# wmeddie/CycloneML

Measured on AMD Instinct MI355X. Metric: rows/s per training iteration, higher is better.
Workload: dtype f64

## Files before the change

### cycloneml_amd/csrc/kmeans.hip

```cpp
#pragma clang fp contract(off)

#include <hip/hip_runtime.h>

#include <algorithm>
#include <cmath>
#include <cstdlib>
#include <mutex>
#include <utility>
#include <vector>

#include "common.hpp"
#include "kmeans_i8.hpp"
#include "kmeans_cos.hpp"
#include "kmeans_fp64.hpp"
#include "kmeans_sparse.hpp"
#include "kmeans_sums.hpp"
#include "silhouette.hpp"

namespace {

using cyc::kmsums::kChunkRows;
using cyc::kmsums::kMaxK;

bool env_is0(const char* name) {
// ... 908 lines not shown
  CYC_REQUIRE(p != nullptr && out != nullptr, "plan and out must not be null");
  CYC_REQUIRE(n >= 0, "n >= 0");
  CYC_REQUIRE(X != nullptr || n == 0, "X must not be null");
  auto* r = new cyc_kmeans_rows_s();
  r->X = X;
  r->n = n;
  r->d = p->d;
  r->usable = p->d <= cyc::km8::kMaxD && p->ktp8 > 0;
  r->cosine = is_cos(p);
  if (r->usable && n > 0) {
    int rc;
    hipStream_t st = cyc::as_stream(stream);
    if ((rc = r->img.reserve((size_t)n * cyc::km8::image_row_bytes(p->d))) ||
        (rc = r->meta.reserve(sizeof(int2) * (size_t)n))) {
      delete r;
      return rc;
    }
    if (r->cosine) {
      cyc::DeviceBuffer xn;
      if ((rc = r->unorm.reserve(sizeof(double) * (size_t)n)) ||
          (rc = xn.reserve(sizeof(double) * (size_t)n))) {
        delete r;
        return rc;
      }
      hipLaunchKernelGGL(k_row_norms, dim3((unsigned)((n + kNormRows - 1) / kNormRows)),
                         dim3(kNormRows), 0, st, X, n, p->d, (double*)xn.ptr);
      CYC_LAUNCH_CHECK("k_row_norms");
      rc = cyc::km8::rows_quantize(X, n, p->d, r->img.ptr, (int2*)r->meta.ptr, st,
                                   (const double*)xn.ptr, (double*)r->unorm.ptr);
      if (!rc && hipStreamSynchronize(st) != hipSuccess) rc = CYC_ERR_HIP;
    } else {
      if ((rc = r->unorm.reserve(sizeof(double) * (size_t)n))) {
        delete r;
        return rc;
      }
      rc = cyc::km8::rows_quantize(X, n, p->d, r->img.ptr, (int2*)r->meta.ptr, st, nullptr,
                                   (double*)r->unorm.ptr);
    }
    if (rc) {
      delete r;
      return rc;
    }
  }
  *out = r;
  return CYC_OK;
}

int cyc_kmeans_rows_destroy(cyc_kmeans_rows rows) {
  delete rows;
  return CYC_OK;
}

int64_t cyc_kmeans_rows_bytes(cyc_kmeans_rows rows) {
  return rows ? (int64_t)(rows->img.bytes + rows->meta.bytes) : 0;
}

int cyc_kmeans_rows_set_bounds(cyc_kmeans_rows rows, int32_t enable) {
  CYC_REQUIRE(rows != nullptr, "rows must not be null");
  rows->bEnabled = enable != 0;
  rows->bValid = false;
  return CYC_OK;
}

int cyc_kmeans_rows_set_incremental(cyc_kmeans_rows rows, int32_t enable) {
  CYC_REQUIRE(rows != nullptr, "rows must not be null");
  rows->inc.enabled = enable != 0;
  rows->inc.valid = false;
  return CYC_OK;
}

int cyc_kmeans_rows_incremental_info(cyc_kmeans_rows rows, int64_t* incremental_calls,
                                     int64_t* moved_rows) {
  CYC_REQUIRE(rows != nullptr && incremental_calls != nullptr && moved_rows != nullptr,
              "arguments must not be null");
  unsigned long long cum[2] = {0, 0};
  if (rows->inc.cum.ptr) {
    CYC_HIP(hipDeviceSynchronize());
    CYC_HIP(hipMemcpy(cum, rows->inc.cum.ptr, sizeof(cum), hipMemcpyDeviceToHost));
  }
  *incremental_calls = (int64_t)cum[1];
  *moved_rows = (int64_t)cum[0];
  return CYC_OK;
}

int cyc_kmeans_rows_bounds_rechecked(cyc_kmeans_rows rows, int64_t* rechecked_rows) {
  CYC_REQUIRE(rows != nullptr && rechecked_rows != nullptr, "arguments must not be null");
  unsigned long long cum = 0;
  if (rows->bRcCum.ptr) {
    CYC_HIP(hipDeviceSynchronize());
    CYC_HIP(hipMemcpy(&cum, rows->bRcCum.ptr, sizeof(cum), hipMemcpyDeviceToHost));
  }
  *rechecked_rows = (int64_t)cum;
  return CYC_OK;
}

int cyc_kmeans_rows_bounds_info(cyc_kmeans_rows rows, int64_t* calls, int64_t* screened_rows) {
  CYC_REQUIRE(rows != nullptr && calls != nullptr && screened_rows != nullptr,
              "arguments must not be null");
  unsigned long long cum = 0;
  if (rows->bCum.ptr) {
    CYC_HIP(hipDeviceSynchronize());
    CYC_HIP(hipMemcpy(&cum, rows->bCum.ptr, sizeof(cum), hipMemcpyDeviceToHost));
  }
  *calls = rows->bCalls;
  *screened_rows = rows->bFullRows + (int64_t)cum;
  return CYC_OK;
}
// ... 420 lines not shown
```

### cycloneml_amd/csrc/kmeans_sums.hip

```cpp
#pragma clang fp contract(off)

#include <hip/hip_runtime.h>

#include <algorithm>
#include <type_traits>

#include "common.hpp"
#include "kmeans_cos.hpp"
#include "kmeans_sums.hpp"

namespace {

constexpr int kSortTile = 4096;
using cyc::kmsums::kChunkRows;

__global__ void k_hist(const int32_t* __restrict__ assign, int64_t n, int k,
                       int32_t* __restrict__ hist, const int* __restrict__ gate) {
  if (gate && !*gate) return;
  extern __shared__ int32_t cnt[];
  for (int c = threadIdx.x; c < k; c += blockDim.x) cnt[c] = 0;
  __syncthreads();
  const int64_t r0 = (int64_t)blockIdx.x * kSortTile;
  const int64_t r1 = min<int64_t>(n, r0 + kSortTile);
  for (int64_t r = r0 + threadIdx.x; r < r1; r += blockDim.x) atomicAdd(&cnt[assign[r]], 1);
  __syncthreads();
  for (int c = threadIdx.x; c < k; c += blockDim.x) hist[(int64_t)blockIdx.x * k + c] = cnt[c];
}

constexpr int kScanSegs = 64;

__global__ void k_scan_seg(const int32_t* __restrict__ hist, int tiles, int k, int segT,
                           int32_t* __restrict__ segsum, const int* __restrict__ gate) {
  if (gate && !*gate) return;
  const int c = blockIdx.x * 64 + threadIdx.x, s = blockIdx.y;
  if (c >= k) return;
  const int t0 = s * segT, t1 = min(tiles, t0 + segT);
  int sum = 0;
#pragma unroll 8
  for (int t = t0; t < t1; ++t) sum += hist[(int64_t)t * k + c];
  segsum[(int64_t)s * k + c] = sum;
}

__global__ void k_scan_segoff(int32_t* __restrict__ segsum, int segs, int k,
                              int64_t* __restrict__ total, const int* __restrict__ gate) {
  if (gate && !*gate) return;
  const int c = blockIdx.x * blockDim.x + threadIdx.x;
  if (c >= k) return;
  int64_t run = 0;
  for (int s = 0; s < segs; ++s) {
    const int32_t h = segsum[(int64_t)s * k + c];
    segsum[(int64_t)s * k + c] = (int32_t)run;
    run += h;
  }
  total[c] = run;
}

__global__ void k_scan_apply(int32_t* __restrict__ hist, int tiles, int k, int segT,
                             const int32_t* __restrict__ segoff, const int* __restrict__ gate) {
  if (gate && !*gate) return;
  const int c = blockIdx.x * 64 + threadIdx.x, s = blockIdx.y;
  if (c >= k) return;
  const int t0 = s * segT, t1 = min(tiles, t0 + segT);
  int32_t run = segoff[(int64_t)s * k + c];
  for (int t = t0; t < t1; ++t) {
    const int32_t h = hist[(int64_t)t * k + c];
    hist[(int64_t)t * k + c] = run;
    run += h;
  }
}

__global__ void k_scan_clusters(const int64_t* __restrict__ total, int k,
                                int64_t* __restrict__ cstart, int64_t* __restrict__ chunkStart,
                                const int* __restrict__ gate) {
  if (gate && !*gate) return;
  __shared__ int64_t s_rows[1024], s_chunks[1024];
  const int tid = threadIdx.x;
  const int per = (k + 1023) / 1024;
  int64_t rows = 0, chunks = 0;
  for (int q = 0; q < per; ++q) {
    int c = tid * per + q;
    if (c < k) {
      rows += total[c];
      chunks += (total[c] + kChunkRows - 1) / kChunkRows;
    }
  }
  s_rows[tid] = rows;
  s_chunks[tid] = chunks;
  __syncthreads();
  for (int off = 1; off < 1024; off <<= 1) {
    int64_t a = tid >= off ? s_rows[tid - off] : 0, b = tid >= off ? s_chunks[tid - off] : 0;
    __syncthreads();
    s_rows[tid] += a;
    s_chunks[tid] += b;
    __syncthreads();
  }
  int64_t rbase = tid ? s_rows[tid - 1] : 0, cbase = tid ? s_chunks[tid - 1] : 0;
  for (int q = 0; q < per; ++q) {
    int c = tid * per + q;
    if (c < k) {
      cstart[c] = rbase;
      chunkStart[c] = cbase;
      rbase += total[c];
      cbase += (total[c] + kChunkRows - 1) / kChunkRows;
    }
  }
  if (tid == 1023) {
    cstart[k] = s_rows[1023];
    chunkStart[k] = s_chunks[1023];
  }
}

__global__ void k_scatter(const int32_t* __restrict__ assign, int64_t n, int k,
                          const int32_t* __restrict__ tileOff, const int64_t* __restrict__ cstart,
                          int32_t* __restrict__ perm, int64_t tiles, const int* __restrict__ gate) {
  if (gate && !*gate) return;
  extern __shared__ int64_t pos[];
  const int64_t per = ((int64_t)gridDim.x + 7) / 8;
  const int64_t tile = (int64_t)(blockIdx.x & 7) * per + (blockIdx.x >> 3);
  if (tile >= tiles) return;
  const int lane = threadIdx.x;
  const int kb = 32 - __builtin_clz((unsigned)max(k - 1, 1));
  for (int c = lane; c < k; c += 64) pos[c] = cstart[c] + tileOff[tile * k + c];
  __syncthreads();
  const int64_t r0 = tile * kSortTile;
  const int64_t r1 = min<int64_t>(n, r0 + kSortTile);
  constexpr int PER = kSortTile / 64;
  int cv[PER];
#pragma unroll
  for (int i = 0; i < PER; ++i) {
    const int64_t r = r0 + i * 64 + lane;
    cv[i] = (r < r1) ? assign[r] : -1;
  }
#pragma unroll
  for (int i = 0; i < PER; ++i) {
    const int64_t r = r0 + i * 64 + lane;
    const int c = cv[i];
    unsigned long long m = __ballot(c >= 0);
    for (int b = 0; b < kb; ++b) {
      const bool bit = (c >> b) & 1;
      const unsigned long long bal = __ballot(bit);
      m &= bit ? bal : ~bal;
    }
    const int prior = __popcll(m & ((1ull << lane) - 1));
    const int last = 63 - __clzll(m);
    int64_t p = (c >= 0) ? pos[c] + prior : 0;
    __builtin_amdgcn_wave_barrier();
    if (c >= 0) {
      perm[p] = (int32_t)r;
      if (last == lane) pos[c] = p + 1;
    }
    __builtin_amdgcn_wave_barrier();
  }
}

template <int NJ>
__global__ __launch_bounds__(256) void k_chunk_sums(
    const double* __restrict__ X, int d, const double* __restrict__ w,
    const double* __restrict__ C, const int32_t* __restrict__ perm,
    const int64_t* __restrict__ cstart, const int64_t* __restrict__ chunkStart, int k,
    double* __restrict__ part, double* __restrict__ pw, double* __restrict__ pc,
    double* __restrict__ costOut) {
// ... 147 lines not shown
      for (int i = 0; i < cnt; ++i) sw = dadd(sw, w[rowsS[i]]);
    } else {
      sw = (double)cnt;
    }
    pw[ch] = sw;
    pc[ch] = red[0];
    if (pa) pa[ch] = reda[0];
  }
}

__global__ void k_chunk_sums_nocost(const double* __restrict__ X, int d,
                                    const double* __restrict__ w,
                                    const double* __restrict__ cost,
                                    const int32_t* __restrict__ perm,
                                    const int64_t* __restrict__ cstart,
                                    const int64_t* __restrict__ chunkStart, int k,
                                    double* __restrict__ part, double* __restrict__ pw,
                                    double* __restrict__ pc) {
  const int64_t ch = blockIdx.x;
  if (ch >= chunkStart[k]) return;
  int lo = 0, hi = k;
  while (hi - lo > 1) {
    int mid = (lo + hi) >> 1;
    if (chunkStart[mid] <= ch) lo = mid; else hi = mid;
  }
  const int c = lo;
  const int64_t first = cstart[c] + (ch - chunkStart[c]) * kChunkRows;
  const int64_t last = min<int64_t>(cstart[c + 1], first + kChunkRows);
  for (int j = threadIdx.x; j < d; j += blockDim.x) {
    double s = 0.0;
    if (w) {
      for (int64_t p = first; p < last; ++p) {
        const int64_t r = perm[p];
        s = dadd(s, dmul(w[r], X[r * d + j]));
      }
    } else {
      for (int64_t p = first; p < last; ++p) s = dadd(s, X[(int64_t)perm[p] * d + j]);
    }
    part[ch * d + j] = s;
  }
  if (threadIdx.x == 0) {
    double sw = 0.0, sc = 0.0;
    for (int64_t p = first; p < last; ++p) {
      const int64_t r = perm[p];
      const double wt = w ? w[r] : 1.0;
      sw = dadd(sw, wt);
      sc = dadd(sc, dmul(cost[r], wt));
    }
    pw[ch] = sw;
    pc[ch] = sc;
  }
}

__global__ void k_reduce_clusters(const double* __restrict__ part, const double* __restrict__ pw,
                                  const double* __restrict__ pc,
                                  const int64_t* __restrict__ chunkStart, int d,
                                  double* __restrict__ sums, double* __restrict__ wsum,
                                  double* __restrict__ ccost, const double* __restrict__ pa,
                                  double* __restrict__ fS, double* __restrict__ fW,
                                  double* __restrict__ fA, const int* __restrict__ gate) {
  if (gate && !*gate) return;
  const int c = blockIdx.x;
  const int64_t a = chunkStart[c], b = chunkStart[c + 1];
  if (a == b) {
    if (threadIdx.x == 0) ccost[c] = 0.0;
    if (fS) {
      for (int j = threadIdx.x; j < d; j += blockDim.x) fS[(int64_t)c * d + j] = 0.0;
      if (threadIdx.x == 0) fW[c] = fA[c] = 0.0;
    }
    return;
  }
  for (int j = threadIdx.x; j < d; j += blockDim.x) {
    double s = 0.0;
    int64_t ch = a;
    for (; ch + 16 <= b; ch += 16) {
      double v[16];
#pragma unroll
      for (int u = 0; u < 16; ++u) v[u] = part[(ch + u) * d + j];
#pragma unroll
      for (int u = 0; u < 16; ++u) s = dadd(s, v[u]);
    }
    for (; ch < b; ++ch) s = dadd(s, part[ch * d + j]);
    sums[(int64_t)c * d + j] = dadd(sums[(int64_t)c * d + j], s);
    if (fS) fS[(int64_t)c * d + j] = s;
  }
  const int tw = 64 % blockDim.x, tc = 128 % blockDim.x, ta = 192 % blockDim.x;
  if (fS && threadIdx.x == ta && ta != tw && ta != tc) {
    double s = 0.0;
    for (int64_t ch = a; ch < b; ++ch) s = dadd(s, pa[ch]);
    fA[c] = s;
  }
  if (threadIdx.x == tw || threadIdx.x == tc) {
    const double* src = threadIdx.x == tw ? pw : pc;
    double s = 0.0;
    int64_t ch = a;
    for (; ch + 8 <= b; ch += 8) {
      double v[8];
#pragma unroll
      for (int u = 0; u < 8; ++u) v[u] = src[ch + u];
#pragma unroll
      for (int u = 0; u < 8; ++u) s = dadd(s, v[u]);
    }
    for (; ch < b; ++ch) s = dadd(s, src[ch]);
    if (threadIdx.x == tw) {
      wsum[c] = dadd(wsum[c], s);
      if (fS) fW[c] = s;
    } else {
      ccost[c] = s;
    }
  }
}

__global__ void k_cost_total(const double* __restrict__ ccost, int k, double* __restrict__ out,
                             const int* __restrict__ gate) {
  if (gate && !*gate) return;
  __shared__ double s[256];
  double a = 0.0;
  for (int c = threadIdx.x; c < k; c += 256) a = dadd(a, ccost[c]);
  s[threadIdx.x] = a;
  __syncthreads();
  for (int off = 128; off > 0; off >>= 1) {
    if (threadIdx.x < off) s[threadIdx.x] = dadd(s[threadIdx.x], s[threadIdx.x + off]);
    __syncthreads();
  }
  if (threadIdx.x == 0) out[0] = dadd(out[0], s[0]);
}

constexpr int kIncRows = 2048;
constexpr int kIncMovedFrac = 16;

__global__ __launch_bounds__(256) void k_inc_moved(const int32_t* __restrict__ assign,
                                                   int32_t* __restrict__ prev, int64_t n,
                                                   int32_t* __restrict__ tmpRow,
                                                   int32_t* __restrict__ tmpOld,
                                                   unsigned int* __restrict__ bcount) {
  constexpr int IT = kIncRows / 256;
  __shared__ unsigned wc[IT * 4];
  const int tid = threadIdx.x, lane = tid & 63, wave = tid >> 6;
  const int64_t base = (int64_t)blockIdx.x * kIncRows;
  unsigned long long masks[IT];
  int32_t olds[IT];
#pragma unroll
  for (int it = 0; it < IT; ++it) {
    const int64_t r = base + it * 256 + tid;
    bool moved = false;
    olds[it] = -1;
    if (r < n) {
      const int32_t a = assign[r], b = prev[r];
      moved = a != b;
      olds[it] = b;
      if (moved) prev[r] = a;
    }
    masks[it] = __builtin_amdgcn_ballot_w64(moved);
    if (lane == 0) wc[it * 4 + wave] = (unsigned)__builtin_popcountll(masks[it]);
  }
  __syncthreads();
  const unsigned long long below = (1ull << lane) - 1ull;
#pragma unroll
  for (int it = 0; it < IT; ++it) {
    unsigned before = 0;
    for (int j = 0; j < it * 4 + wave; ++j) before += wc[j];
    if ((masks[it] >> lane) & 1ull) {
      const int64_t pos = base + before + (unsigned)__builtin_popcountll(masks[it] & below);
      tmpRow[pos] = (int32_t)(base + it * 256 + tid);
      tmpOld[pos] = olds[it];
    }
  }
  if (tid == 0) {
    unsigned total = 0;
    for (int j = 0; j < IT * 4; ++j) total += wc[j];
    bcount[blockIdx.x] = total;
  }
}

__global__ __launch_bounds__(1024) void k_inc_scan(unsigned int* __restrict__ bcount, int64_t nb,
                                                   unsigned int* __restrict__ count, int valid,
                                                   int64_t mcap, int* __restrict__ gate,
                                                   unsigned long long* __restrict__ movedCum) {
// ... 17 lines not shown
    bcount[i] = run;
    run += c;
  }
  if (t == 1023) {
    const unsigned total = part[1023];
    bcount[nb] = total;
    *count = total;
    const int inc = valid && (int64_t)total <= mcap;
    gate[0] = inc ? 0 : 1;
    gate[1] = inc ? 1 : 0;
    if (inc) *movedCum += (unsigned long long)total;
  }
}

__global__ __launch_bounds__(256) void k_inc_gather(const int32_t* __restrict__ tmpRow,
                                                    const int32_t* __restrict__ tmpOld,
                                                    const unsigned int* __restrict__ bcount,
                                                    const int32_t* __restrict__ assign,
                                                    int32_t* __restrict__ movedRow,
                                                    int32_t* __restrict__ movedNew,
                                                    int32_t* __restrict__ movedOld,
                                                    const int* __restrict__ gate) {
  if (!gate[1]) return;
  const int64_t b = blockIdx.x, base = b * kIncRows;
  const unsigned off = bcount[b], cnt = bcount[b + 1] - off;
  for (unsigned i = threadIdx.x; i < cnt; i += 256) {
    const int32_t r = tmpRow[base + i];
    movedRow[off + i] = r;
    movedNew[off + i] = assign[r];
    movedOld[off + i] = tmpOld[base + i];
  }
}

template <int NV>
__device__ __forceinline__ void inc_block_sum(double (&v)[NV], double* red) {
  const int tid = threadIdx.x;
  __syncthreads();
#pragma unroll
  for (int i = 0; i < NV; ++i) red[i * 256 + tid] = v[i];
  __syncthreads();
  for (int off = 128; off > 0; off >>= 1) {
    if (tid < off) {
#pragma unroll
      for (int i = 0; i < NV; ++i) red[i * 256 + tid] = dadd(red[i * 256 + tid], red[i * 256 + tid + off]);
    }
    __syncthreads();
  }
#pragma unroll
  for (int i = 0; i < NV; ++i) v[i] = red[i * 256];
}

constexpr int kIncScan = 8;
constexpr int kIncSplit = 8;
constexpr int kIncPs = 6;
template <int NJ>
__global__ __launch_bounds__(256) void k_inc_part(
    const double* __restrict__ X, int d, const double* __restrict__ xnorm,
    const int32_t* __restrict__ movedRow, const int32_t* __restrict__ movedNew,
    const int32_t* __restrict__ movedOld, const unsigned int* __restrict__ count,
    const double* __restrict__ P, double* __restrict__ pds, double* __restrict__ psc,
    const int* __restrict__ gate) {
  if (!gate[1]) return;
  constexpr int B = 256 * kIncScan;
  __shared__ int32_t rowsS[B];
  __shared__ float sgS[B];
  __shared__ unsigned wcS[kIncScan * 4];
  __shared__ double red[5 * 256];
  const int c = blockIdx.x, g = blockIdx.y, tid = threadIdx.x, lane = tid & 63, wave = tid >> 6;
  const unsigned m = *count;
  const unsigned s0 = (unsigned)((uint64_t)m * g / kIncSplit);
  const unsigned s1 = (unsigned)((uint64_t)m * (g + 1) / kIncSplit);
  int64_t ent = 0;
  double ds[NJ], dq[NJ], dqa[NJ], pj[NJ];
#pragma unroll
  for (int u = 0; u < NJ; ++u) {
    const int j = tid + 256 * u;
    ds[u] = dq[u] = dqa[u] = 0.0;
    pj[u] = j < d ? P[(int64_t)c * d + j] : 0.0;
  }
  double tN = 0.0, tA = 0.0, tAbs = 0.0;
  const unsigned long long below = (1ull << lane) - 1ull;
  for (unsigned base = s0; base < s1; base += B) {
    int nw[kIncScan], ol[kIncScan];
#pragma unroll
    for (int q = 0; q < kIncScan; ++q) {
      const unsigned i = base + q * 256 + tid;
      nw[q] = i < s1 ? movedNew[i] : -1;
      ol[q] = i < s1 ? movedOld[i] : -1;
    }
    unsigned long long mk[kIncScan];
    __syncthreads();
#pragma unroll
    for (int q = 0; q < kIncScan; ++q) {
      mk[q] = __builtin_amdgcn_ballot_w64(nw[q] == c || ol[q] == c);
      if (lane == 0) wcS[q * 4 + wave] = (unsigned)__builtin_popcountll(mk[q]);
    }
    __syncthreads();
    int cnt = 0;
#pragma unroll
    for (int q = 0; q < kIncScan; ++q) {
      unsigned before = 0;
      for (int j = 0; j < q * 4 + wave; ++j) before += wcS[j];
      if ((mk[q] >> lane) & 1ull) {
        const unsigned pos = before + (unsigned)__builtin_popcountll(mk[q] & below);
        rowsS[pos] = movedRow[base + q * 256 + tid];
        sgS[pos] = nw[q] == c ? 1.0f : -1.0f;
      }
    }
    for (int j = 0; j < kIncScan * 4; ++j) cnt += (int)wcS[j];
    __syncthreads();
    ent += cnt;
    for (int e = tid; e < cnt; e += 256) {
      const bool add = sgS[e] > 0.0f;
      const double xn = xnorm[rowsS[e]];
      tN += add ? 1.0 : -1.0;
      tA = add ? dadd(tA, xn) : dsub(tA, xn);
      tAbs = dadd(tAbs, xn);
    }
    for (int p0 = 0; p0 < cnt; p0 += 8) {
      double xv[8][NJ];
#pragma unroll
      for (int v = 0; v < 8; ++v) {
        const int64_t r = rowsS[min(p0 + v, cnt - 1)];
#pragma unroll
        for (int u = 0; u < NJ; ++u) {
          const int j = tid + 256 * u;
          xv[v][u] = j < d ? X[r * d + j] : 0.0;
        }
      }
#pragma unroll
      for (int v = 0; v < 8; ++v) {
        if (p0 + v < cnt) {
          const bool add = sgS[p0 + v] > 0.0f;
#pragma unroll
          for (int u = 0; u < NJ; ++u) {
            const double x = xv[v][u];
            const double df = dsub(pj[u], x);
            const double t = dmul(df, df);
            ds[u] = add ? dadd(ds[u], x) : dsub(ds[u], x);
            dq[u] = add ? dadd(dq[u], t) : dsub(dq[u], t);
            dqa[u] = dadd(dqa[u], t);
          }
        }
      }
    }
  }
  double r1[5] = {0.0, 0.0, tN, tA, tAbs};
#pragma unroll
  for (int u = 0; u < NJ; ++u) {
    r1[0] = dadd(r1[0], dq[u]);
    r1[1] = dadd(r1[1], dqa[u]);
  }
  inc_block_sum<5>(r1, red);
  const int64_t slot = (int64_t)c * kIncSplit + g;
#pragma unroll
  for (int u = 0; u < NJ; ++u) {
    const int j = tid + 256 * u;
    if (j < d) pds[slot * d + j] = ds[u];
  }
  if (tid < 5) psc[slot * kIncPs + tid] = r1[tid];
  if (tid == 5) psc[slot * kIncPs + 5] = (double)ent;
}
// ... 153 lines not shown
  const int c = blockIdx.x, lane = threadIdx.x;
  const double w = wsum[c];
  if (!(w > 0)) return;
  const double a = 1.0 / w;
  double* crow = C + (int64_t)c * d;
  const double* srow = sums + (int64_t)c * d;
  if (d > kUpdLds) {
    if (lane == 0) {
      double moved = 0.0, nn = 0.0;
      for (int j = 0; j < d; ++j) {
        const double v = dmul(a, srow[j]);
        const double sc = dsub(v, crow[j]);
        moved = dadd(moved, dmul(sc, sc));
        nn = dadd(nn, dmul(v, v));
      }
      cnorm[c] = __builtin_sqrt(nn);
      if (!(moved <= eps2) && converged) atomicAnd(converged, 0);
    }
    __syncthreads();
    for (int j = lane; j < d; j += 64) crow[j] = dmul(a, srow[j]);
    return;
  }
  for (int j = lane; j < d; j += 64) {
    const double v = dmul(a, srow[j]);
    const double sc = dsub(v, crow[j]);
    upd[j] = dmul(sc, sc);
    upd[d + j] = dmul(v, v);
    crow[j] = v;
  }
  __syncthreads();
  if (lane == 0) {
    double moved = 0.0, nn = 0.0;
    for (int j = 0; j < d; ++j) {
      moved = dadd(moved, upd[j]);
      nn = dadd(nn, upd[d + j]);
    }
    cnorm[c] = __builtin_sqrt(nn);
    if (!(moved <= eps2) && converged) atomicAnd(converged, 0);
  }
}

template <class F>
void with_nj(int nj, F&& f) {
  if (nj == 1) f(std::integral_constant<int, 1>{});
  else if (nj == 2) f(std::integral_constant<int, 2>{});
  else f(std::integral_constant<int, 4>{});
}

}

namespace cyc {
namespace kmsums {

int sort_clusters(SortScratch& s, const int32_t* assign, int64_t n, int d, int k, hipStream_t st,
                  int64_t& maxChunks, const int* gate) {
  int rc;
  const int tiles = (int)((n + kSortTile - 1) / kSortTile);
  maxChunks = (n + kChunkRows - 1) / kChunkRows + k;
  if ((rc = s.hist.reserve(sizeof(int32_t) * (size_t)tiles * k)) ||
      (rc = s.total.reserve(sizeof(int64_t) * (size_t)k)) ||
      (rc = s.cstart.reserve(sizeof(int64_t) * (size_t)(k + 1))) ||
      (rc = s.chunkStart.reserve(sizeof(int64_t) * (size_t)(k + 1))) ||
      (rc = s.perm.reserve(sizeof(int32_t) * (size_t)n)) ||
      (rc = s.part.reserve(sizeof(double) * (size_t)maxChunks * d)) ||
      (rc = s.pw.reserve(sizeof(double) * (size_t)maxChunks)) ||
      (rc = s.pc.reserve(sizeof(double) * (size_t)maxChunks)) ||
      (rc = s.ccost.reserve(sizeof(double) * (size_t)k)))
    return rc;
  int32_t* hist = (int32_t*)s.hist.ptr;
  hipLaunchKernelGGL(k_hist, dim3(tiles), dim3(256), sizeof(int32_t) * k, st, assign, n, k, hist,
                     gate);
  CYC_LAUNCH_CHECK("k_hist");
  {
    const int segT = (tiles + std::min(kScanSegs, tiles) - 1) / std::min(kScanSegs, tiles);
    const int segs = (tiles + segT - 1) / segT;
    if ((rc = s.segsum.reserve(sizeof(int32_t) * (size_t)segs * k))) return rc;
    int32_t* segsum = (int32_t*)s.segsum.ptr;
    hipLaunchKernelGGL(k_scan_seg, dim3((unsigned)((k + 63) / 64), (unsigned)segs), dim3(64), 0, st,
                       (const int32_t*)hist, tiles, k, segT, segsum, gate);
    CYC_LAUNCH_CHECK("k_scan_seg");
    hipLaunchKernelGGL(k_scan_segoff, dim3((unsigned)((k + 255) / 256)), dim3(256), 0, st, segsum,
                       segs, k, (int64_t*)s.total.ptr, gate);
    CYC_LAUNCH_CHECK("k_scan_segoff");
    hipLaunchKernelGGL(k_scan_apply, dim3((unsigned)((k + 63) / 64), (unsigned)segs), dim3(64), 0,
                       st, hist, tiles, k, segT, (const int32_t*)segsum, gate);
    CYC_LAUNCH_CHECK("k_scan_apply");
  }
  hipLaunchKernelGGL(k_scan_clusters, dim3(1), dim3(1024), 0, st, (const int64_t*)s.total.ptr, k,
                     (int64_t*)s.cstart.ptr, (int64_t*)s.chunkStart.ptr, gate);
  CYC_LAUNCH_CHECK("k_scan_clusters");
  hipLaunchKernelGGL(k_scatter, dim3((unsigned)(8 * (((int64_t)tiles + 7) / 8))), dim3(64),
                     sizeof(int64_t) * k, st, assign, n, k, hist, (const int64_t*)s.cstart.ptr,
                     (int32_t*)s.perm.ptr, (int64_t)tiles, gate);
  CYC_LAUNCH_CHECK("k_scatter");
  return CYC_OK;
}

int full_pass(SortScratch& s, const double* X, int64_t n, int d, int k, const double* weights,
              const double* xnorm, bool cosine, const double* C, const int32_t* assign,
              double* cost, double* sums, double* wsum, double* cost_sum, hipStream_t st,
              const int* gate, IncState* inc) {
  const int nj = (d + 255) / 256;
  int rc;
  int64_t maxChunks = 0;
  if ((rc = sort_clusters(s, assign, n, d, k, st, maxChunks, gate))) return rc;
  if (inc && (rc = inc->pa.reserve(sizeof(double) * (size_t)maxChunks))) return rc;
  const int32_t* perm = (const int32_t*)s.perm.ptr;
  const int64_t* cstart = (const int64_t*)s.cstart.ptr;
  const int64_t* chunkStart = (const int64_t*)s.chunkStart.ptr;
  double *part = (double*)s.part.ptr, *pw = (double*)s.pw.ptr, *pc = (double*)s.pc.ptr;
  double* pa = inc ? (double*)inc->pa.ptr : nullptr;
  if (cosine) {
    if ((rc = cyc::kmcos::chunk_sums(X, d, weights, xnorm, cost, perm, cstart, chunkStart, k,
                                     maxChunks, part, pw, pc, st)))
      return rc;
  } else {
    cyc::KernelTimer timer("k_chunk_sums", st);
    const dim3 grid((unsigned)maxChunks);
    if (!cost && nj <= 4)
      with_nj(nj, [&](auto NJ) {
        hipLaunchKernelGGL(HIP_KERNEL_NAME(k_chunk_sums_fast<decltype(NJ)::value>), grid,
                           dim3(256), 0, st, X, d, weights, C, perm, cstart, chunkStart, k, part,
                           pw, pc, inc ? xnorm : (const double*)nullptr, pa, gate);
      });
    else if (nj <= 4)
      with_nj(nj, [&](auto NJ) {
        hipLaunchKernelGGL(HIP_KERNEL_NAME(k_chunk_sums<decltype(NJ)::value>), grid, dim3(256), 0,
                           st, X, d, weights, C, perm, cstart, chunkStart, k, part, pw, pc,
                           cost);
      });
    else
      hipLaunchKernelGGL(k_chunk_sums_nocost, grid, dim3(256), 0, st, X, d, weights,
                         (const double*)cost, perm, cstart, chunkStart, k, part, pw, pc);
    CYC_LAUNCH_CHECK("k_chunk_sums");
  }
  hipLaunchKernelGGL(k_reduce_clusters, dim3(k), dim3(256), 0, st, (const double*)part,
                     (const double*)pw, (const double*)pc, chunkStart, d, sums, wsum,
                     (double*)s.ccost.ptr, (const double*)pa,
                     inc ? (double*)inc->S.ptr : nullptr, inc ? (double*)inc->W.ptr : nullptr,
                     inc ? (double*)inc->A.ptr : nullptr, gate);
  CYC_LAUNCH_CHECK("k_reduce_clusters");
  hipLaunchKernelGGL(k_cost_total, dim3(1), dim3(256), 0, st, (const double*)s.ccost.ptr, k,
                     cost_sum, gate);
  CYC_LAUNCH_CHECK("k_cost_total");
  return CYC_OK;
}

int inc_accumulate(SortScratch& s, IncState& inc, const double* X, const double* xnorm,
                   const int32_t* assign, int64_t n, int d, int k, const double* C, double* sums,
                   double* wsum, double* cost_sum, hipStream_t st) {
  const int nj = (d + 255) / 256;
  const int64_t nb = (n + kIncRows - 1) / kIncRows;
  const int64_t mcap = n / kIncMovedFrac;
  const size_t kd = (size_t)k * d;
  int rc;
  const bool fresh = inc.prev.ptr == nullptr;
  if ((rc = inc.prev.reserve(sizeof(int32_t) * (size_t)n)) ||
      (rc = inc.tmpRow.reserve(sizeof(int32_t) * (size_t)n)) ||
      (rc = inc.tmpOld.reserve(sizeof(int32_t) * (size_t)n)) ||
      (rc = inc.bcount.reserve(sizeof(unsigned int) * (size_t)(nb + 1))) ||
      (rc = inc.count.reserve(64)) || (rc = inc.gate.reserve(64)) ||
      (rc = inc.movedRow.reserve(sizeof(int32_t) * (size_t)std::max<int64_t>(mcap, 1))) ||
      (rc = inc.movedNew.reserve(sizeof(int32_t) * (size_t)std::max<int64_t>(mcap, 1))) ||
      (rc = inc.movedOld.reserve(sizeof(int32_t) * (size_t)std::max<int64_t>(mcap, 1))) ||
      (rc = inc.S.reserve(sizeof(double) * kd)) || (rc = inc.P.reserve(sizeof(double) * kd)) ||
      (rc = inc.pds.reserve(sizeof(double) * kd * kIncSplit)) ||
      (rc = inc.psc.reserve(sizeof(double) * (size_t)k * kIncSplit * kIncPs)) ||
      (rc = inc.W.reserve(sizeof(double) * (size_t)k)) ||
      (rc = inc.Q.reserve(sizeof(double) * (size_t)k)) ||
      (rc = inc.N.reserve(sizeof(int64_t) * (size_t)k)) ||
      (rc = inc.A.reserve(sizeof(double) * (size_t)k)) ||
      (rc = inc.ES.reserve(sizeof(double) * (size_t)k)) ||
      (rc = inc.EQ.reserve(sizeof(double) * (size_t)k)) ||
      (rc = inc.cost.reserve(sizeof(double) * (size_t)k)) ||
      (rc = inc.err.reserve(sizeof(double) * (size_t)k)) ||
      (rc = inc.bad.reserve(sizeof(int) * (size_t)k)) || (rc = inc.tot.reserve(64)) ||
      (rc = inc.cum.reserve(64)))
    return rc;
  if (fresh) {
    CYC_HIP(hipMemsetAsync(inc.prev.ptr, 0xff, sizeof(int32_t) * (size_t)n, st));
    CYC_HIP(hipMemsetAsync(inc.cum.ptr, 0, 16, st));
  }
  const int valid = inc.valid && inc.k == k ? 1 : 0;
  inc.valid = false;
  int* gate = (int*)inc.gate.ptr;
  unsigned long long* cum = (unsigned long long*)inc.cum.ptr;
  const unsigned int* cnt = (const unsigned int*)inc.count.ptr;
  {
    cyc::KernelTimer timer("k_kmeans_inc", st);
    hipLaunchKernelGGL(k_inc_moved, dim3((unsigned)nb), dim3(256), 0, st, assign,
                       (int32_t*)inc.prev.ptr, n, (int32_t*)inc.tmpRow.ptr,
                       (int32_t*)inc.tmpOld.ptr, (unsigned int*)inc.bcount.ptr);
    CYC_LAUNCH_CHECK("k_inc_moved");
    hipLaunchKernelGGL(k_inc_scan, dim3(1), dim3(1024), 0, st, (unsigned int*)inc.bcount.ptr,
                       nb, (unsigned int*)inc.count.ptr, valid, mcap, gate, cum);
    CYC_LAUNCH_CHECK("k_inc_scan");
    hipLaunchKernelGGL(k_inc_gather, dim3((unsigned)nb), dim3(256), 0, st,
                       (const int32_t*)inc.tmpRow.ptr, (const int32_t*)inc.tmpOld.ptr,
                       (const unsigned int*)inc.bcount.ptr, assign,
                       (int32_t*)inc.movedRow.ptr, (int32_t*)inc.movedNew.ptr,
                       (int32_t*)inc.movedOld.ptr, (const int*)gate);
    CYC_LAUNCH_CHECK("k_inc_gather");
    with_nj(nj, [&](auto NJ) {
      constexpr int J = decltype(NJ)::value;
      hipLaunchKernelGGL(HIP_KERNEL_NAME(k_inc_part<J>), dim3((unsigned)k, kIncSplit), dim3(256),
                         0, st, X, d, xnorm, (const int32_t*)inc.movedRow.ptr,
                         (const int32_t*)inc.movedNew.ptr, (const int32_t*)inc.movedOld.ptr, cnt,
                         (const double*)inc.P.ptr, (double*)inc.pds.ptr, (double*)inc.psc.ptr,
                         (const int*)gate);
      hipLaunchKernelGGL(HIP_KERNEL_NAME(k_inc_combine<J>), dim3((unsigned)k), dim3(256), 0, st,
                         d, C, (const double*)inc.pds.ptr, (const double*)inc.psc.ptr,
                         (double*)inc.S.ptr, (const double*)inc.P.ptr, (double*)inc.W.ptr,
                         (double*)inc.Q.ptr, (int64_t*)inc.N.ptr, (double*)inc.A.ptr,
                         (double*)inc.ES.ptr, (double*)inc.EQ.ptr, (double*)inc.cost.ptr,
                         (double*)inc.err.ptr, (int*)inc.bad.ptr, (const int*)gate);
    });
    CYC_LAUNCH_CHECK("k_inc_part / k_inc_combine");
    hipLaunchKernelGGL(k_inc_check, dim3(1), dim3(256), 0, st, (const double*)inc.cost.ptr,
                       (const double*)inc.err.ptr, (const int*)inc.bad.ptr, k, gate,
                       (double*)inc.tot.ptr, cum + 1);
    CYC_LAUNCH_CHECK("k_inc_check");
  }
  if ((rc = full_pass(s, X, n, d, k, nullptr, xnorm, false, C, assign, nullptr, sums, wsum,
                      cost_sum, st, gate, &inc)))
    return rc;
  hipLaunchKernelGGL(k_inc_finish, dim3(k), dim3(256), 0, st, C, d, (double*)inc.P.ptr,
                     (const double*)s.ccost.ptr, (const int64_t*)s.total.ptr,
                     (const int64_t*)s.chunkStart.ptr, (double*)inc.Q.ptr,
                     (int64_t*)inc.N.ptr, (const double*)inc.A.ptr, (double*)inc.ES.ptr,
                     (double*)inc.EQ.ptr, (const double*)inc.S.ptr,
                     (const double*)inc.W.ptr, (const double*)inc.tot.ptr, sums, wsum,
                     cost_sum, (const int*)gate);
  CYC_LAUNCH_CHECK("k_inc_finish");
  return CYC_OK;
}

int update_centers(double* C, double* cnorm, const double* sums, const double* wsum, int k, int d,
                   double eps2, int32_t* converged, hipStream_t st) {
  hipLaunchKernelGGL(k_update_centers, dim3((unsigned)k), dim3(64),
                     d <= kUpdLds ? sizeof(double) * 2 * (size_t)d : 0, st, C, cnorm, sums, wsum,
                     k, d, eps2, converged);
  CYC_LAUNCH_CHECK("k_update_centers");
  return CYC_OK;
}

}
}
```

### cycloneml_amd/csrc/kmeans_sums.hpp

```cpp
#pragma once

#include <hip/hip_runtime.h>

#include <cstdint>

#include "common.hpp"

namespace cyc {
namespace kmsums {

constexpr int kChunkRows = 256;
constexpr int kMaxK = 8192;

struct SortScratch {
  DeviceBuffer hist, total, cstart, chunkStart, perm, part, pw, pc, ccost, segsum;
};

struct IncState {
  bool enabled = true;
  bool valid = false;
  int k = 0;
  DeviceBuffer prev, tmpRow, tmpOld, bcount, count, gate, movedRow, movedNew, movedOld, S, P, W,
      Q, N, A, ES, EQ, cost, err, bad, tot, cum, pa, pds, psc;
};

int sort_clusters(SortScratch& s, const int32_t* assign, int64_t n, int d, int k, hipStream_t st,
                  int64_t& maxChunks, const int* gate = nullptr);

int full_pass(SortScratch& s, const double* X, int64_t n, int d, int k, const double* weights,
              const double* xnorm, bool cosine, const double* C, const int32_t* assign,
              double* cost, double* sums, double* wsum, double* cost_sum, hipStream_t st,
              const int* gate = nullptr, IncState* inc = nullptr);

int inc_accumulate(SortScratch& s, IncState& inc, const double* X, const double* xnorm,
                   const int32_t* assign, int64_t n, int d, int k, const double* C, double* sums,
                   double* wsum, double* cost_sum, hipStream_t st);

int update_centers(double* C, double* cnorm, const double* sums, const double* wsum, int k, int d,
                   double eps2, int32_t* converged, hipStream_t st);

}
}
```

Baseline: 14.28 billion.

## Fuse scan and cost-total kernels via last-block pattern; pre-bucket moved rows per cluster

Several small kernels are merged into their predecessors with a last-workgroup atomic counter: the segment-offset scan and cluster scan now run inside k_scan_seg, and the cost total runs inside k_reduce_clusters. This cuts kernel launches and serialization points per iteration. A new k_inc_index kernel buckets moved rows by cluster once, using a shared-memory histogram and a stable ordering, so k_inc_part reads only its own cluster's records instead of ballot-scanning every moved row for every cluster. The price is extra scratch buffers, a device-side counter that has to reset correctly, and reliance on fences for cross-block visibility.

```diff
diff --git a/cycloneml_amd/csrc/kmeans.hip b/cycloneml_amd/csrc/kmeans.hip
--- a/cycloneml_amd/csrc/kmeans.hip
+++ b/cycloneml_amd/csrc/kmeans.hip
@@ -984,7 +984,7 @@
 }
 
 int64_t cyc_kmeans_rows_bytes(cyc_kmeans_rows rows) {
-  return rows ? (int64_t)(rows->img.bytes + rows->meta.bytes) : 0;
+  return rows ? (int64_t)(rows->img.bytes + rows->meta.bytes + rows->inc.bytes()) : 0;
 }
 
 int cyc_kmeans_rows_set_bounds(cyc_kmeans_rows rows, int32_t enable) {
diff --git a/cycloneml_amd/csrc/kmeans_sums.hip b/cycloneml_amd/csrc/kmeans_sums.hip
--- a/cycloneml_amd/csrc/kmeans_sums.hip
+++ b/cycloneml_amd/csrc/kmeans_sums.hip
@@ -27,32 +27,97 @@
   for (int c = threadIdx.x; c < k; c += blockDim.x) hist[(int64_t)blockIdx.x * k + c] = cnt[c];
 }
 
+__device__ __forceinline__ bool last_workgroup(unsigned int* counter, unsigned total) {
+  __shared__ unsigned s_last;
+  asm volatile("s_waitcnt vmcnt(0)" ::: "memory");
+  __syncthreads();
+  if (threadIdx.x == 0) {
+    __threadfence();
+    asm volatile("s_waitcnt vmcnt(0)" ::: "memory");
+    const unsigned t = __hip_atomic_fetch_add(counter, 1u, __ATOMIC_RELAXED, __HIP_MEMORY_SCOPE_AGENT);
+    const unsigned last = t == total - 1 ? 1u : 0u;
+    if (last) {
+      __threadfence();
+      asm volatile("s_waitcnt vmcnt(0)" ::: "memory");
+      *counter = 0u;
+    }
+    s_last = last;
+  }
+  __syncthreads();
+  return s_last != 0u;
+}
+
 constexpr int kScanSegs = 64;
 
-__global__ void k_scan_seg(const int32_t* __restrict__ hist, int tiles, int k, int segT,
-                           int32_t* __restrict__ segsum, const int* __restrict__ gate) {
+__device__ __forceinline__ void scan_segoff_clusters(int32_t* segsum, int segs, int k,
+                                                     int64_t* __restrict__ total,
+                                                     int64_t* __restrict__ cstart,
+                                                     int64_t* __restrict__ chunkStart) {
+  __shared__ int64_t s_rows[256], s_chunks[256];
+  const int tid = threadIdx.x;
+  for (int c = tid; c < k; c += 256) {
+    int64_t run = 0;
+    for (int s = 0; s < segs; ++s) {
+      const int32_t h = segsum[(int64_t)s * k + c];
+      segsum[(int64_t)s * k + c] = (int32_t)run;
+      run += h;
+    }
+    total[c] = run;
+  }
+  __syncthreads();
+  const int per = (k + 255) / 256;
+  int64_t rows = 0, chunks = 0;
+  for (int q = 0; q < per; ++q) {
+    const int c = tid * per + q;
+    if (c < k) {
+      rows += total[c];
+      chunks += (total[c] + kChunkRows - 1) / kChunkRows;
+    }
+  }
+  s_rows[tid] = rows;
+  s_chunks[tid] = chunks;
+  __syncthreads();
+  for (int off = 1; off < 256; off <<= 1) {
+    int64_t a = tid >= off ? s_rows[tid - off] : 0, b = tid >= off ? s_chunks[tid - off] : 0;
+    __syncthreads();
+    s_rows[tid] += a;
+    s_chunks[tid] += b;
+    __syncthreads();
+  }
+  int64_t rbase = tid ? s_rows[tid - 1] : 0, cbase = tid ? s_chunks[tid - 1] : 0;
+  for (int q = 0; q < per; ++q) {
+    const int c = tid * per + q;
+    if (c < k) {
+      cstart[c] = rbase;
+      chunkStart[c] = cbase;
+      rbase += total[c];
+      cbase += (total[c] + kChunkRows - 1) / kChunkRows;
+    }
+  }
+  if (tid == 255) {
+    cstart[k] = s_rows[255];
+    chunkStart[k] = s_chunks[255];
+  }
+}
+
+__global__ __launch_bounds__(256) void k_scan_seg(const int32_t* __restrict__ hist, int tiles, int k,
+                                                  int segT, int32_t* segsum, int segs,
+                                                  int64_t* __restrict__ total,
+                                                  int64_t* __restrict__ cstart,
+                                                  int64_t* __restrict__ chunkStart,
+                                                  unsigned int* __restrict__ done,
+                                                  const int* __restrict__ gate) {
   if (gate && !*gate) return;
-  const int c = blockIdx.x * 64 + threadIdx.x, s = blockIdx.y;
-  if (c >= k) return;
-  const int t0 = s * segT, t1 = min(tiles, t0 + segT);
-  int sum = 0;
+  const int c = blockIdx.x * 256 + threadIdx.x, s = blockIdx.y;
+  if (c < k) {
+    const int t0 = s * segT, t1 = min(tiles, t0 + segT);
+    int sum = 0;
 #pragma unroll 8
-  for (int t = t0; t < t1; ++t) sum += hist[(int64_t)t * k + c];
-  segsum[(int64_t)s * k + c] = sum;
-}
-
-__global__ void k_scan_segoff(int32_t* __restrict__ segsum, int segs, int k,
-                              int64_t* __restrict__ total, const int* __restrict__ gate) {
-  if (gate && !*gate) return;
-  const int c = blockIdx.x * blockDim.x + threadIdx.x;
-  if (c >= k) return;
-  int64_t run = 0;
-  for (int s = 0; s < segs; ++s) {
-    const int32_t h = segsum[(int64_t)s * k + c];
-    segsum[(int64_t)s * k + c] = (int32_t)run;
-    run += h;
-  }
-  total[c] = run;
+    for (int t = t0; t < t1; ++t) sum += hist[(int64_t)t * k + c];
+    segsum[(int64_t)s * k + c] = sum;
+  }
+  if (last_workgroup(done, gridDim.x * gridDim.y))
+    scan_segoff_clusters(segsum, segs, k, total, cstart, chunkStart);
 }
 
 __global__ void k_scan_apply(int32_t* __restrict__ hist, int tiles, int k, int segT,
@@ -66,47 +131,6 @@
     const int32_t h = hist[(int64_t)t * k + c];
     hist[(int64_t)t * k + c] = run;
     run += h;
-  }
-}
-
-__global__ void k_scan_clusters(const int64_t* __restrict__ total, int k,
-                                int64_t* __restrict__ cstart, int64_t* __restrict__ chunkStart,
-                                const int* __restrict__ gate) {
-  if (gate && !*gate) return;
-  __shared__ int64_t s_rows[1024], s_chunks[1024];
-  const int tid = threadIdx.x;
-  const int per = (k + 1023) / 1024;
-  int64_t rows = 0, chunks = 0;
-  for (int q = 0; q < per; ++q) {
-    int c = tid * per + q;
-    if (c < k) {
-      rows += total[c];
-      chunks += (total[c] + kChunkRows - 1) / kChunkRows;
-    }
-  }
-  s_rows[tid] = rows;
-  s_chunks[tid] = chunks;
-  __syncthreads();
-  for (int off = 1; off < 1024; off <<= 1) {
-    int64_t a = tid >= off ? s_rows[tid - off] : 0, b = tid >= off ? s_chunks[tid - off] : 0;
-    __syncthreads();
-    s_rows[tid] += a;
-    s_chunks[tid] += b;
-    __syncthreads();
-  }
-  int64_t rbase = tid ? s_rows[tid - 1] : 0, cbase = tid ? s_chunks[tid - 1] : 0;
-  for (int q = 0; q < per; ++q) {
-    int c = tid * per + q;
-    if (c < k) {
-      cstart[c] = rbase;
-      chunkStart[c] = cbase;
-      rbase += total[c];
-      cbase += (total[c] + kChunkRows - 1) / kChunkRows;
-    }
-  }
-  if (tid == 1023) {
-    cstart[k] = s_rows[1023];
-    chunkStart[k] = s_chunks[1023];
   }
 }
 
@@ -360,14 +384,24 @@
   }
 }
 
-__global__ void k_reduce_clusters(const double* __restrict__ part, const double* __restrict__ pw,
-                                  const double* __restrict__ pc,
-                                  const int64_t* __restrict__ chunkStart, int d,
-                                  double* __restrict__ sums, double* __restrict__ wsum,
-                                  double* __restrict__ ccost, const double* __restrict__ pa,
-                                  double* __restrict__ fS, double* __restrict__ fW,
-                                  double* __restrict__ fA, const int* __restrict__ gate) {
-  if (gate && !*gate) return;
+__device__ __forceinline__ void cost_total(const double* ccost, int k, double* __restrict__ out) {
+  __shared__ double s[256];
+  double a = 0.0;
+  for (int c = threadIdx.x; c < k; c += 256) a = dadd(a, ccost[c]);
+  s[threadIdx.x] = a;
+  __syncthreads();
+  for (int off = 128; off > 0; off >>= 1) {
+    if (threadIdx.x < off) s[threadIdx.x] = dadd(s[threadIdx.x], s[threadIdx.x + off]);
+    __syncthreads();
+  }
+  if (threadIdx.x == 0) out[0] = dadd(out[0], s[0]);
+}
+
+__device__ __forceinline__ void reduce_cluster(
+    const double* __restrict__ part, const double* __restrict__ pw, const double* __restrict__ pc,
+    const int64_t* __restrict__ chunkStart, int d, double* __restrict__ sums,
+    double* __restrict__ wsum, double* ccost, const double* __restrict__ pa,
+    double* __restrict__ fS, double* __restrict__ fW, double* __restrict__ fA) {
   const int c = blockIdx.x;
   const int64_t a = chunkStart[c], b = chunkStart[c + 1];
   if (a == b) {
@@ -419,19 +453,15 @@
   }
 }
 
-__global__ void k_cost_total(const double* __restrict__ ccost, int k, double* __restrict__ out,
-                             const int* __restrict__ gate) {
+__global__ __launch_bounds__(256) void k_reduce_clusters(
+    const double* __restrict__ part, const double* __restrict__ pw, const double* __restrict__ pc,
+    const int64_t* __restrict__ chunkStart, int d, double* __restrict__ sums,
+    double* __restrict__ wsum, double* ccost, const double* __restrict__ pa,
+    double* __restrict__ fS, double* __restrict__ fW, double* __restrict__ fA, int k,
+    double* __restrict__ costSum, unsigned int* __restrict__ done, const int* __restrict__ gate) {
   if (gate && !*gate) return;
-  __shared__ double s[256];
-  double a = 0.0;
-  for (int c = threadIdx.x; c < k; c += 256) a = dadd(a, ccost[c]);
-  s[threadIdx.x] = a;
-  __syncthreads();
-  for (int off = 128; off > 0; off >>= 1) {
-    if (threadIdx.x < off) s[threadIdx.x] = dadd(s[threadIdx.x], s[threadIdx.x + off]);
-    __syncthreads();
-  }
-  if (threadIdx.x == 0) out[0] = dadd(out[0], s[0]);
+  reduce_cluster(part, pw, pc, chunkStart, d, sums, wsum, ccost, pa, fS, fW, fA);
+  if (last_workgroup(done, gridDim.x)) cost_total(ccost, k, costSum);
 }
 
 constexpr int kIncRows = 2048;
@@ -555,21 +585,103 @@
 
 constexpr int kIncScan = 8;
 constexpr int kIncSplit = 8;
+constexpr int kIncBatch = 256 * kIncScan;
+__global__ __launch_bounds__(256) void k_inc_index(const int32_t* __restrict__ movedRow,
+                                                   const int32_t* __restrict__ movedNew,
+                                                   const int32_t* __restrict__ movedOld,
+                                                   const unsigned int* __restrict__ count, int k,
+                                                   int bmax, int32_t* __restrict__ boff,
+                                                   int32_t* __restrict__ recs,
+                                                   const int* __restrict__ gate) {
+  if (!gate[1]) return;
+  constexpr int B = kIncBatch;
+  extern __shared__ int32_t hs[];
+  __shared__ int32_t keyS[2 * B];
+  __shared__ int32_t scanS[256];
+  const int g = blockIdx.y, tid = threadIdx.x;
+  const unsigned m = *count;
+  const unsigned s0 = (unsigned)((uint64_t)m * g / kIncSplit);
+  const unsigned s1 = (unsigned)((uint64_t)m * (g + 1) / kIncSplit);
+  const uint64_t base64 = (uint64_t)s0 + (uint64_t)blockIdx.x * B;
+  if (base64 >= s1) return;
+  const unsigned base = (unsigned)base64;
+  int nw[kIncScan], ol[kIncScan], rw[kIncScan];
+#pragma unroll
+  for (int q = 0; q < kIncScan; ++q) {
+    const unsigned i = base + q * 256 + tid;
+    const bool in = i < s1;
+    nw[q] = in ? movedNew[i] : -1;
+    ol[q] = in ? movedOld[i] : -1;
+    rw[q] = in ? movedRow[i] : 0;
+    if ((unsigned)nw[q] >= (unsigned)k) nw[q] = -1;
+    if ((unsigned)ol[q] >= (unsigned)k) ol[q] = -1;
+  }
+  for (int c = tid; c < k; c += 256) hs[c] = 0;
+  __syncthreads();
+#pragma unroll
+  for (int q = 0; q < kIncScan; ++q) {
+    if (nw[q] >= 0) atomicAdd(&hs[nw[q]], 1);
+    if (ol[q] >= 0) atomicAdd(&hs[ol[q]], 1);
+  }
+  __syncthreads();
+  const int per = (k + 255) / 256;
+  const int c0 = min(k, tid * per), c1 = min(k, c0 + per);
+  int sum = 0;
+  for (int c = c0; c < c1; ++c) sum += hs[c];
+  scanS[tid] = sum;
+  __syncthreads();
+  for (int off = 1; off < 256; off <<= 1) {
+    const int v = tid >= off ? scanS[tid - off] : 0;
+    __syncthreads();
+    scanS[tid] += v;
+    __syncthreads();
+  }
+  int32_t* const bo = boff + ((int64_t)g * bmax + blockIdx.x) * (k + 1);
+  int run = tid ? scanS[tid - 1] : 0;
+  for (int c = c0; c < c1; ++c) {
+    const int h = hs[c];
+    hs[c] = run;
+    bo[c] = run;
+    run += h;
+  }
+  if (tid == 255) bo[k] = scanS[255];
+  __syncthreads();
+#pragma unroll
+  for (int q = 0; q < kIncScan; ++q) {
+    const int e = q * 256 + tid;
+    if (nw[q] >= 0) keyS[atomicAdd(&hs[nw[q]], 1)] = 2 * e;
+    if (ol[q] >= 0) keyS[atomicAdd(&hs[ol[q]], 1)] = 2 * e + 1;
+  }
+  __syncthreads();
+  int32_t* const out = recs + 2 * (int64_t)base;
+#pragma unroll
+  for (int q = 0; q < kIncScan; ++q) {
+    const int e = q * 256 + tid;
+#pragma unroll
+    for (int side = 0; side < 2; ++side) {
+      const int c = side ? ol[q] : nw[q];
+      if (c < 0) continue;
+      const int a = c ? hs[c - 1] : 0, b = hs[c], key = 2 * e + side;
+      int rank = 0;
+      for (int j = a; j < b; ++j) rank += keyS[j] < key ? 1 : 0;
+      out[a + rank] = side ? ~rw[q] : rw[q];
+    }
+  }
+}
+
 constexpr int kIncPs = 6;
 template <int NJ>
 __global__ __launch_bounds__(256) void k_inc_part(
     const double* __restrict__ X, int d, const double* __restrict__ xnorm,
-    const int32_t* __restrict__ movedRow, const int32_t* __restrict__ movedNew,
-    const int32_t* __restrict__ movedOld, const unsigned int* __restrict__ count,
-    const double* __restrict__ P, double* __restrict__ pds, double* __restrict__ psc,
-    const int* __restrict__ gate) {
+    const int32_t* __restrict__ boff, const int32_t* __restrict__ recs, int k, int bmax,
+    const unsigned int* __restrict__ count, const double* __restrict__ P,
+    double* __restrict__ pds, double* __restrict__ psc, const int* __restrict__ gate) {
   if (!gate[1]) return;
-  constexpr int B = 256 * kIncScan;
+  constexpr int B = kIncBatch;
   __shared__ int32_t rowsS[B];
   __shared__ float sgS[B];
-  __shared__ unsigned wcS[kIncScan * 4];
   __shared__ double red[5 * 256];
-  const int c = blockIdx.x, g = blockIdx.y, tid = threadIdx.x, lane = tid & 63, wave = tid >> 6;
+  const int c = blockIdx.x, g = blockIdx.y, tid = threadIdx.x;
   const unsigned m = *count;
   const unsigned s0 = (unsigned)((uint64_t)m * g / kIncSplit);
   const unsigned s1 = (unsigned)((uint64_t)m * (g + 1) / kIncSplit);
@@ -582,35 +694,17 @@
     pj[u] = j < d ? P[(int64_t)c * d + j] : 0.0;
   }
   double tN = 0.0, tA = 0.0, tAbs = 0.0;
-  const unsigned long long below = (1ull << lane) - 1ull;
-  for (unsigned base = s0; base < s1; base += B) {
-    int nw[kIncScan], ol[kIncScan];
-#pragma unroll
-    for (int q = 0; q < kIncScan; ++q) {
-      const unsigned i = base + q * 256 + tid;
-      nw[q] = i < s1 ? movedNew[i] : -1;
-      ol[q] = i < s1 ? movedOld[i] : -1;
-    }
-    unsigned long long mk[kIncScan];
-    __syncthreads();
-#pragma unroll
-    for (int q = 0; q < kIncScan; ++q) {
-      mk[q] = __builtin_amdgcn_ballot_w64(nw[q] == c || ol[q] == c);
-      if (lane == 0) wcS[q * 4 + wave] = (unsigned)__builtin_popcountll(mk[q]);
-    }
-    __syncthreads();
-    int cnt = 0;
-#pragma unroll
-    for (int q = 0; q < kIncScan; ++q) {
-      unsigned before = 0;
-      for (int j = 0; j < q * 4 + wave; ++j) before += wcS[j];
-      if ((mk[q] >> lane) & 1ull) {
-        const unsigned pos = before + (unsigned)__builtin_popcountll(mk[q] & below);
-        rowsS[pos] = movedRow[base + q * 256 + tid];
-        sgS[pos] = nw[q] == c ? 1.0f : -1.0f;
-      }
-    }
-    for (int j = 0; j < kIncScan * 4; ++j) cnt += (int)wcS[j];
+  const int32_t* bo = boff + (int64_t)g * bmax * (k + 1) + c;
+  for (uint64_t base = s0; base < s1; base += B, bo += k + 1) {
+    const int a = bo[0], cnt = bo[1] - a;
+    if (cnt == 0) continue;
+    const int32_t* rec = recs + 2 * (int64_t)base + a;
+    __syncthreads();
+    for (int e = tid; e < cnt; e += 256) {
+      const int32_t r = rec[e];
+      rowsS[e] = r < 0 ? ~r : r;
+      sgS[e] = r < 0 ? -1.0f : 1.0f;
+    }
     __syncthreads();
     ent += cnt;
     for (int e = tid; e < cnt; e += 256) {
@@ -870,6 +964,14 @@
 namespace cyc {
 namespace kmsums {
 
+static int sync_reserve(SortScratch& s, hipStream_t st) {
+  if (s.sync.ptr) return CYC_OK;
+  int rc;
+  if ((rc = s.sync.reserve(64))) return rc;
+  CYC_HIP(hipMemsetAsync(s.sync.ptr, 0, 64, st));
+  return CYC_OK;
+}
+
 int sort_clusters(SortScratch& s, const int32_t* assign, int64_t n, int d, int k, hipStream_t st,
                   int64_t& maxChunks, const int* gate) {
   int rc;
@@ -885,6 +987,7 @@
       (rc = s.pc.reserve(sizeof(double) * (size_t)maxChunks)) ||
       (rc = s.ccost.reserve(sizeof(double) * (size_t)k)))
     return rc;
+  if ((rc = sync_reserve(s, st))) return rc;
   int32_t* hist = (int32_t*)s.hist.ptr;
   hipLaunchKernelGGL(k_hist, dim3(tiles), dim3(256), sizeof(int32_t) * k, st, assign, n, k, hist,
                      gate);
@@ -894,19 +997,15 @@
     const int segs = (tiles + segT - 1) / segT;
     if ((rc = s.segsum.reserve(sizeof(int32_t) * (size_t)segs * k))) return rc;
     int32_t* segsum = (int32_t*)s.segsum.ptr;
-    hipLaunchKernelGGL(k_scan_seg, dim3((unsigned)((k + 63) / 64), (unsigned)segs), dim3(64), 0, st,
-                       (const int32_t*)hist, tiles, k, segT, segsum, gate);
+    hipLaunchKernelGGL(k_scan_seg, dim3((unsigned)((k + 255) / 256), (unsigned)segs), dim3(256), 0,
+                       st, (const int32_t*)hist, tiles, k, segT, segsum, segs,
+                       (int64_t*)s.total.ptr, (int64_t*)s.cstart.ptr, (int64_t*)s.chunkStart.ptr,
+                       (unsigned int*)s.sync.ptr, gate);
     CYC_LAUNCH_CHECK("k_scan_seg");
-    hipLaunchKernelGGL(k_scan_segoff, dim3((unsigned)((k + 255) / 256)), dim3(256), 0, st, segsum,
-                       segs, k, (int64_t*)s.total.ptr, gate);
-    CYC_LAUNCH_CHECK("k_scan_segoff");
     hipLaunchKernelGGL(k_scan_apply, dim3((unsigned)((k + 63) / 64), (unsigned)segs), dim3(64), 0,
                        st, hist, tiles, k, segT, (const int32_t*)segsum, gate);
     CYC_LAUNCH_CHECK("k_scan_apply");
   }
-  hipLaunchKernelGGL(k_scan_clusters, dim3(1), dim3(1024), 0, st, (const int64_t*)s.total.ptr, k,
-                     (int64_t*)s.cstart.ptr, (int64_t*)s.chunkStart.ptr, gate);
-  CYC_LAUNCH_CHECK("k_scan_clusters");
   hipLaunchKernelGGL(k_scatter, dim3((unsigned)(8 * (((int64_t)tiles + 7) / 8))), dim3(64),
                      sizeof(int64_t) * k, st, assign, n, k, hist, (const int64_t*)s.cstart.ptr,
                      (int32_t*)s.perm.ptr, (int64_t)tiles, gate);
@@ -956,11 +1055,9 @@
                      (const double*)pw, (const double*)pc, chunkStart, d, sums, wsum,
                      (double*)s.ccost.ptr, (const double*)pa,
                      inc ? (double*)inc->S.ptr : nullptr, inc ? (double*)inc->W.ptr : nullptr,
-                     inc ? (double*)inc->A.ptr : nullptr, gate);
+                     inc ? (double*)inc->A.ptr : nullptr, k, cost_sum,
+                     (unsigned int*)s.sync.ptr + 1, gate);
   CYC_LAUNCH_CHECK("k_reduce_clusters");
-  hipLaunchKernelGGL(k_cost_total, dim3(1), dim3(256), 0, st, (const double*)s.ccost.ptr, k,
-                     cost_sum, gate);
-  CYC_LAUNCH_CHECK("k_cost_total");
   return CYC_OK;
 }
 
@@ -970,6 +1067,7 @@
   const int nj = (d + 255) / 256;
   const int64_t nb = (n + kIncRows - 1) / kIncRows;
   const int64_t mcap = n / kIncMovedFrac;
+  const int bmax = (int)(mcap / kIncSplit / kIncBatch + 1);
   const size_t kd = (size_t)k * d;
   int rc;
   const bool fresh = inc.prev.ptr == nullptr;
@@ -981,6 +1079,8 @@
       (rc = inc.movedRow.reserve(sizeof(int32_t) * (size_t)std::max<int64_t>(mcap, 1))) ||
       (rc = inc.movedNew.reserve(sizeof(int32_t) * (size_t)std::max<int64_t>(mcap, 1))) ||
       (rc = inc.movedOld.reserve(sizeof(int32_t) * (size_t)std::max<int64_t>(mcap, 1))) ||
+      (rc = inc.boff.reserve(sizeof(int32_t) * (size_t)kIncSplit * bmax * (k + 1))) ||
+      (rc = inc.recs.reserve(sizeof(int32_t) * 2 * (size_t)std::max<int64_t>(mcap, 1))) ||
       (rc = inc.S.reserve(sizeof(double) * kd)) || (rc = inc.P.reserve(sizeof(double) * kd)) ||
       (rc = inc.pds.reserve(sizeof(double) * kd * kIncSplit)) ||
       (rc = inc.psc.reserve(sizeof(double) * (size_t)k * kIncSplit * kIncPs)) ||
@@ -1019,13 +1119,17 @@
                        (int32_t*)inc.movedRow.ptr, (int32_t*)inc.movedNew.ptr,
                        (int32_t*)inc.movedOld.ptr, (const int*)gate);
     CYC_LAUNCH_CHECK("k_inc_gather");
+    hipLaunchKernelGGL(k_inc_index, dim3((unsigned)bmax, kIncSplit), dim3(256),
+                       sizeof(int32_t) * (size_t)k, st, (const int32_t*)inc.movedRow.ptr,
+                       (const int32_t*)inc.movedNew.ptr, (const int32_t*)inc.movedOld.ptr, cnt, k,
+                       bmax, (int32_t*)inc.boff.ptr, (int32_t*)inc.recs.ptr, (const int*)gate);
+    CYC_LAUNCH_CHECK("k_inc_index");
     with_nj(nj, [&](auto NJ) {
       constexpr int J = decltype(NJ)::value;
       hipLaunchKernelGGL(HIP_KERNEL_NAME(k_inc_part<J>), dim3((unsigned)k, kIncSplit), dim3(256),
-                         0, st, X, d, xnorm, (const int32_t*)inc.movedRow.ptr,
-                         (const int32_t*)inc.movedNew.ptr, (const int32_t*)inc.movedOld.ptr, cnt,
-                         (const double*)inc.P.ptr, (double*)inc.pds.ptr, (double*)inc.psc.ptr,
-                         (const int*)gate);
+                         0, st, X, d, xnorm, (const int32_t*)inc.boff.ptr,
+                         (const int32_t*)inc.recs.ptr, k, bmax, cnt, (const double*)inc.P.ptr,
+                         (double*)inc.pds.ptr, (double*)inc.psc.ptr, (const int*)gate);
       hipLaunchKernelGGL(HIP_KERNEL_NAME(k_inc_combine<J>), dim3((unsigned)k), dim3(256), 0, st,
                          d, C, (const double*)inc.pds.ptr, (const double*)inc.psc.ptr,
                          (double*)inc.S.ptr, (const double*)inc.P.ptr, (double*)inc.W.ptr,
diff --git a/cycloneml_amd/csrc/kmeans_sums.hpp b/cycloneml_amd/csrc/kmeans_sums.hpp
--- a/cycloneml_amd/csrc/kmeans_sums.hpp
+++ b/cycloneml_amd/csrc/kmeans_sums.hpp
@@ -3,6 +3,7 @@
 #include <hip/hip_runtime.h>
 
 #include <cstdint>
+#include <initializer_list>
 
 #include "common.hpp"
 
@@ -13,7 +14,7 @@
 constexpr int kMaxK = 8192;
 
 struct SortScratch {
-  DeviceBuffer hist, total, cstart, chunkStart, perm, part, pw, pc, ccost, segsum;
+  DeviceBuffer hist, total, cstart, chunkStart, perm, part, pw, pc, ccost, segsum, sync;
 };
 
 struct IncState {
@@ -21,7 +22,15 @@
   bool valid = false;
   int k = 0;
   DeviceBuffer prev, tmpRow, tmpOld, bcount, count, gate, movedRow, movedNew, movedOld, S, P, W,
-      Q, N, A, ES, EQ, cost, err, bad, tot, cum, pa, pds, psc;
+      Q, N, A, ES, EQ, cost, err, bad, tot, cum, pa, pds, psc, boff, recs;
+  size_t bytes() const {
+    size_t b = 0;
+    for (const DeviceBuffer* q : {&prev, &tmpRow, &tmpOld, &bcount, &count, &gate, &movedRow,
+                                  &movedNew, &movedOld, &S, &P, &W, &Q, &N, &A, &ES, &EQ, &cost,
+                                  &err, &bad, &tot, &cum, &pa, &pds, &psc, &boff, &recs})
+      b += q->bytes;
+    return b;
+  }
 };
 
 int sort_clusters(SortScratch& s, const int32_t* assign, int64_t n, int d, int k, hipStream_t st,
```

Result: slower. 14.01 billion (-1.9%).
